# arindamrc/video_analytics

Hardware: AMD Instinct MI355X
Metric: clips/sec (224x224, RGB+10-flow two-stream) (higher is better)
Workload: dtype f32; 1 GPU; two-stream 224x224, 10-frame TV-L1 flow stack (5 scales x 5 warps x 300 its, fixed), VGG-16 spatial+temporal, batch=32 per GPU; global_batch=32, block_iters=0, tvl1_math=exact, flow_streams=2, batches_in_flight=1, tvl1_params=, tvl1_hip_blob=08077c666a7db564113fbd6e9b9134d85ffd8245, parallelism=clips sharded x1, finite=True

## Files before the change

video_analytics_amd/csrc/tvl1.hip:

```cpp
#include "va_internal.h"
#include <cmath>
#include <algorithm>
#include <cstdlib>
#include <cstring>
#include <utility>
#include <type_traits>

namespace {

constexpr int kNF_STATE = 6;
constexpr int kNF_RO = 4;


__device__ __forceinline__ void bilinear3_shfl(const float* __restrict__ I1, size_t plane, int w, int h, int pitch, float x,
                                               float y, bool active, float& v0, float& v1, float& v2)
{
    x = fminf(fmaxf(x, 0.0f), (float)(w - 1));
    y = fminf(fmaxf(y, 0.0f), (float)(h - 1));
    const int x0 = (int)x, y0 = (int)y;
    const int x1 = d_min(x0 + 1, w - 1), y1 = d_min(y0 + 1, h - 1);
    const float ax = x - (float)x0, ay = y - (float)y0;
    const int o00 = y0 * pitch + x0, o10 = y1 * pitch + x0;
    float a[3], c[3], b[3], d[3];
#pragma unroll
// ... 30 lines not shown
    v2 = r[2];
}

__global__ void k_warp(const float* __restrict__ pyr, size_t plane, int w, int h, int pitch, int fps,
                       const float* __restrict__ stA, const float* __restrict__ stB, const int* __restrict__ sel, int cur,
                       int* __restrict__ base, float* __restrict__ ro, int pair0, int perm)
{
    unsigned lid = blockIdx.y * gridDim.x + blockIdx.x;
    {
        const unsigned nb = gridDim.x * gridDim.y, q = nb / 8, r = nb % 8, xcd = lid % 8, kk = lid / 8;
        lid = (xcd < r ? xcd * (q + 1) : r * (q + 1) + (xcd - r) * q) + kk;
    }
    const int pair = pair0 + (int)(lid / gridDim.x);
    const int idx = (int)(lid % gridDim.x) * blockDim.x + threadIdx.x;
    const int which = sel ? sel[pair] : cur;
    if (base && idx == 0) base[pair] = which;
    const bool active = idx < w * h;
    const int y = active ? idx / w : 0, x = active ? idx - y * w : 0;
    const int seq = pair / (fps - 1), k = pair - seq * (fps - 1);
    const int f0 = seq * fps + k;
    const float* I0 = pyr + (size_t)f0 * 3 * plane;
    const float* I1 = pyr + (size_t)(f0 + 1) * 3 * plane;
    const float* st = (which ? stB : stA) + (size_t)pair * kNF_STATE * plane;
    const size_t o = (size_t)y * pitch + x, op = (size_t)y * pitch + pslot(x, perm);
    const float u1 = active ? st[op] : 0.0f, u2 = active ? st[plane + op] : 0.0f;
    float Iw, Iwx, Iwy;
    bilinear3_shfl(I1, plane, w, h, pitch, (float)x + u1, (float)y + u2, active, Iw, Iwx, Iwy);
    if (!active) return;
    const float grad = fmaf(Iwy, Iwy, Iwx * Iwx);
    float* r = ro + (size_t)pair * kNF_RO * plane;
    r[op] = Iwx;
    r[plane + op] = Iwy;
    r[2 * plane + op] = fmaf(-Iwy, u2, fmaf(-Iwx, u1, Iw - I0[o]));
    r[3 * plane + op] = grad < 1e-10f ? 0.0f : 1.0f / grad;
}

__global__ void k_upsample(const float* __restrict__ stA, const float* __restrict__ stB, const int* __restrict__ sel,
                           int cur, int cw, int ch, int cpitch, size_t cplane, float* __restrict__ tmp, int fw, int fh,
                           int fpitch, size_t fplane, float inv_step, int cperm)
{
    const int pair = blockIdx.y;
    const int idx = blockIdx.x * blockDim.x + threadIdx.x;
    if (idx >= fw * fh) return;
    const int which = sel ? sel[pair] : cur;
    const float* src = (which ? stB : stA) + (size_t)pair * kNF_STATE * cplane;
    float* dst = tmp + (size_t)pair * 2 * fplane;
    const int y = idx / fw, x = idx - y * fw;
    const float rx = (float)cw / (float)fw, ry = (float)ch / (float)fh;
    const size_t o = (size_t)y * fpitch + x;
    dst[o] = bilinear(src, cw, ch, cpitch, (float)x * rx, (float)y * ry, cperm) * inv_step;
    dst[fplane + o] = bilinear(src + cplane, cw, ch, cpitch, (float)x * rx, (float)y * ry, cperm) * inv_step;
}

__global__ void k_level_init(const float* __restrict__ tmp, float* __restrict__ st0, int w, int h, int pitch, size_t plane, int perm)
{
    const int pair = blockIdx.y;
    const int idx = blockIdx.x * blockDim.x + threadIdx.x;
    if (idx >= pitch * h) return;
    const int y = idx / pitch, x = idx - y * pitch;
    const size_t o = (size_t)y * pitch + x, op = (size_t)y * pitch + pslot(x, perm);
    const float* t = tmp + (size_t)pair * 2 * plane;
    float* dst = st0 + (size_t)pair * kNF_STATE * plane;
    dst[op] = x < w ? t[o] : 0.0f;
    dst[plane + op] = x < w ? t[plane + o] : 0.0f;
    dst[2 * plane + op] = 0.0f;
    dst[3 * plane + op] = 0.0f;
    dst[4 * plane + op] = 0.0f;
    dst[5 * plane + op] = 0.0f;
}

__global__ void k_zero_pad(float* __restrict__ buf, int nf, int w, int h, int pitch, size_t plane, int perm)
{
    const int pair = blockIdx.y, pw = pitch - w;
    const int idx = blockIdx.x * blockDim.x + threadIdx.x;
    if (idx >= pw * h * nf) return;
    const int f = idx / (pw * h), r = idx - f * pw * h, y = r / pw, x = w + r - y * pw;
    buf[((size_t)pair * nf + f) * plane + (size_t)y * pitch + pslot(x, perm)] = 0.0f;
}

__global__ void k_flow_out(const float* __restrict__ stA, const float* __restrict__ stB, const int* __restrict__ sel,
                           int cur, int w, int h, int pitch, size_t plane, float* __restrict__ flow, int perm)
{
    const int pair = blockIdx.y;
    const int idx = blockIdx.x * blockDim.x + threadIdx.x;
    if (idx >= w * h) return;
    const int which = sel ? sel[pair] : cur;
    const float* st = (which ? stB : stA) + (size_t)pair * kNF_STATE * plane;
    const int y = idx / w, x = idx - y * w;
    flow[((size_t)pair * 2) * w * h + idx] = st[(size_t)y * pitch + pslot(x, perm)];
    flow[((size_t)pair * 2 + 1) * w * h + idx] = st[plane + (size_t)y * pitch + pslot(x, perm)];
}

__global__ void k_flow_to_stack(const float* __restrict__ flow, float* __restrict__ stack, size_t n, float bound,
                                float mean, float stdv)
{
    const size_t i = (size_t)blockIdx.x * blockDim.x + threadIdx.x;
    if (i >= n) return;
    const float t = (255.0f * (flow[i] + bound)) / (2.0f * bound);
    const float q = rintf(fminf(fmaxf(t, 0.0f), 255.0f));
    stack[i] = (q / 255.0f - mean) / stdv;
}


struct IterArgs {
    const float* ro;
    const float* stA;
    const float* stB;
    float* outA;
    float* outB;
    const int* base;
    int* sel;
    unsigned long long* err;
    unsigned long long qthr;
// ... 387 lines not shown
    float prev = dpp_from_left(row_get(a, N - 1));
#pragma clang loop unroll(full)
    for (int i = 0; i < N; ++i) {
        const float cur = row_get(a, i);
        row_set(d, i, i == 0 ? cur - prev : sub_s(cur, prev));
        prev = cur;
    }
    return d;
}
template <int N>
__device__ __forceinline__ Row<N> r_diff_fwd(const Row<N>& a)
{
    Row<N> d;
    d.t = 0.0f;
    const float right = dpp_from_right(row_get(a, 0));
#pragma clang loop unroll(full)
    for (int i = 0; i < N; ++i)
        row_set(d, i, i < N - 1 ? sub_s(row_get(a, i + 1 < N ? i + 1 : 0), row_get(a, i)) : right - row_get(a, i));
    return d;
}

template <int PPL> struct RowIo;
template <> struct RowIo<2> {
    typedef unsigned V __attribute__((ext_vector_type(2)));
    static __device__ __forceinline__ V ld(__amdgpu_buffer_rsrc_t r, int vo, int so) { return __builtin_amdgcn_raw_buffer_load_b64(r, vo, so, 0); }
    static __device__ __forceinline__ void st(V v, __amdgpu_buffer_rsrc_t r, int vo, int so) { __builtin_amdgcn_raw_buffer_store_b64(v, r, vo, so, 0); }
};
template <int N>
__device__ __forceinline__ Row<N> row_load(__amdgpu_buffer_rsrc_t r, int vo, int so)
{
    const typename RowIo<N>::V v = RowIo<N>::ld(r, vo, so);
    Row<N> o;
    o.t = 0.0f;
#pragma clang loop unroll(full)
    for (int i = 0; i < N; ++i) row_set(o, i, __uint_as_float(v[i]));
    return o;
}
template <int N>
__device__ __forceinline__ void row_store(const Row<N>& o, __amdgpu_buffer_rsrc_t r, int vo, int so)
{
    typename RowIo<N>::V v;
#pragma clang loop unroll(full)
    for (int i = 0; i < N; ++i) v[i] = __float_as_uint(row_get(o, i));
    RowIo<N>::st(v, r, vo, so);
}


struct StreamArgs {
    const float* ro;
    const float* sin;
    float* sout;
    size_t plane;
    int w, h, pitch;
    int nsx, nch, R, HX;
    int K;
    int pair0, rev;
    float l_t, taut, theta;
    int narrow, npairs;
};

template <int KH, int NCH>
struct StreamShape {
    static_assert(KH % NCH == 0, "the levels of a wave are cut into chains of equal length");
    static constexpr int KC = KH / NCH;
    static constexpr int SPAN = KH + NCH;
    static constexpr int lpos(int t) { return t + t / KC; }
// ... 19 lines not shown
    typedef StreamRow<PPL> SR;
    typedef StreamShape<KH, NCH> SH;
    constexpr int NP = R::NP, NT = R::NT, SW = 64 * PPL, KC = SH::KC;
    constexpr int NRING = stream_ring_rows<KH, NWV, NCH>() > 0 ? stream_ring_rows<KH, NWV, NCH>() : 1;
    typedef float f4 __attribute__((ext_vector_type(4)));
    static_assert(kNF_RO % 2 == 0 && kNF_STATE % 2 == 0, "fields pair up into 16-byte units");
    __shared__ f4 ringP[NRING][kNF_RO / 2][NP][64];
    __shared__ float ringT[NRING][kNF_RO][NT ? 64 : 1];
    __shared__ f4 ifaceP[NWV > 1 ? NWV - 1 : 1][2][kNF_STATE / 2][NP][64];
    __shared__ float ifaceT[NWV > 1 ? NWV - 1 : 1][2][kNF_STATE][NT ? 64 : 1];

    const int sx = job % a.nsx, ch = job / a.nsx;
    const int w = a.w, h = a.h, pitch = a.pitch;
    const int lane = threadIdx.x & 63;
    const int wv = NWV == 1 ? 0 : __builtin_amdgcn_readfirstlane((int)(threadIdx.x >> 6));
    const int ox = sx * (SW - 2 * a.HX);
    const int vx0 = ox + (sx > 0 ? a.HX : 0), vx1 = (sx == a.nsx - 1) ? pitch : ox + SW - a.HX;
    const int x0 = ox + PPL * (half ? (lane & 31) : lane);
    const bool colok = x0 < pitch && !(half == 2 && lane >= 32);
    const bool stok = colok && x0 >= vx0 && x0 < vx1;
    const int a0 = ch * a.R, b0 = d_min(h, a0 + a.R);
    const int ys = d_max(0, a0 - K), ye = d_min(h, b0 + K);

    const int planeb = (int)(a.plane * sizeof(float)), pitchb = pitch * (int)sizeof(float);
    const int npr = half == 1 ? 2 : 1;
    const __amdgpu_buffer_rsrc_t rs_ro = __builtin_amdgcn_make_buffer_rsrc(
        const_cast<float*>(a.ro + (size_t)pair * kNF_RO * a.plane), 0, npr * kNF_RO * planeb, 0x00020000);
    const __amdgpu_buffer_rsrc_t rs_in = __builtin_amdgcn_make_buffer_rsrc(
        const_cast<float*>(sin_all + (size_t)pair * kNF_STATE * a.plane), 0, npr * kNF_STATE * planeb, 0x00020000);
    const __amdgpu_buffer_rsrc_t rs_out = __builtin_amdgcn_make_buffer_rsrc(sout_all + (size_t)pair * kNF_STATE * a.plane, 0,
                                                                           npr * kNF_STATE * planeb, 0x00020000);
    const bool second = half == 1 && lane >= 32;
    const int loff = colok ? x0 * (int)sizeof(float) + (second ? kNF_STATE * planeb : 0) : 0;
    const int loff_ro = colok ? x0 * (int)sizeof(float) + (second ? kNF_RO * planeb : 0) : 0;

    R mx;
    mx.t = 0.0f;
#pragma clang loop unroll(full)
    for (int i = 0; i < PPL; ++i) row_set(mx, i, x0 + i < w - 1 ? 1.0f : 0.0f);
    const float l_t = a.l_t, taut = a.taut, theta = a.theta;
    const R zero = row_splat<PPL>(0.0f), one = row_splat<PPL>(1.0f);

    auto unit_put = [&](f4 (*u)[64], float (*t)[NT ? 64 : 1], int f, const R& v0, const R& v1) __attribute__((always_inline)) {
#pragma clang loop unroll(full)
        for (int j = 0; j < NP; ++j) u[j][lane] = f4{v0.p[j].x, v0.p[j].y, v1.p[j].x, v1.p[j].y};
        if constexpr (NT) {
            t[f][lane] = v0.t;
            t[f + 1][lane] = v1.t;
        }
    };
    auto unit_get = [&](const f4 (*u)[64], const float (*t)[NT ? 64 : 1], int f, R& v0, R& v1) __attribute__((always_inline)) {
#pragma clang loop unroll(full)
        for (int j = 0; j < NP; ++j) {
            const f4 q = u[j][lane];
            v0.p[j] = f2{q.x, q.y};
            v1.p[j] = f2{q.z, q.w};
        }
// ... 15 lines not shown
        unit_put(ifaceP[wb][b][0], ifaceT[wb][b], 0, v.u1, v.u2);
        unit_put(ifaceP[wb][b][1], ifaceT[wb][b], 2, v.p11, v.p12);
        unit_put(ifaceP[wb][b][2], ifaceT[wb][b], 4, v.p21, v.p22);
    };
    auto if_get = [&](int wb, int b, SR& v) __attribute__((always_inline)) {
        unit_get(ifaceP[wb][b][0], ifaceT[wb][b], 0, v.u1, v.u2);
        unit_get(ifaceP[wb][b][1], ifaceT[wb][b], 2, v.p11, v.p12);
        unit_get(ifaceP[wb][b][2], ifaceT[wb][b], 4, v.p21, v.p22);
    };

    {
        const R zro[kNF_RO] = {zero, zero, zero, zero};
        for (int r = wv; r < NRING; r += NWV) ring_put(r, zro);
    }
    if constexpr (NWV > 1) {
        if (wv < NWV - 1) {
            const SR zst{zero, zero, zero, zero, zero, zero};
            if_put(wv, 0, zst);
            if_put(wv, 1, zst);
        }
        __syncthreads();
    }

    auto ld = [&](const __amdgpu_buffer_rsrc_t& r, int f, int y) -> R { return row_load<PPL>(r, loff, f * planeb + y * pitchb); };
    auto ld_ro = [&](int f, int y) -> R { return row_load<PPL>(rs_ro, loff_ro, f * planeb + y * pitchb); };
    auto st = [&](const R& v, int f, int y) { row_store<PPL>(v, rs_out, loff, f * planeb + y * pitchb); };

    const int nsteps = b0 - ys + K + (NWV * NCH - 1);

    auto run = [&](auto wave_tag, auto mx1_tag) __attribute__((always_inline)) {
        constexpr int W = decltype(wave_tag)::value;
        constexpr bool MX1 = decltype(mx1_tag)::value;
        constexpr bool FIRST = W == 0, LAST = W == NWV - 1;
        constexpr int G0 = W * KH, LAG = W * SH::SPAN;

        R P11[KH], P12[KH], P21[KH], P22[KH], U1[KH], U2[KH];
#pragma clang loop unroll(full)
        for (int t = 0; t < KH; ++t) P11[t] = P12[t] = P21[t] = P22[t] = U1[t] = U2[t] = zero;
        SR latch[NCH > 1 ? NCH - 1 : 1];
#pragma clang loop unroll(full)
        for (int c = 0; c < (NCH > 1 ? NCH - 1 : 1); ++c) latch[c] = SR{zero, zero, zero, zero, zero, zero};
        R nst[kNF_STATE], nro[kNF_RO], rprev[kNF_RO] = {zero, zero, zero, zero};
        constexpr bool KEEP = LAST && stream_keep_last<KH, NWV, NCH>();
        R keep[kNF_RO] = {zero, zero, zero, zero};
#pragma clang loop unroll(full)
        for (int f = 0; f < kNF_STATE; ++f) nst[f] = FIRST ? ld(rs_in, f, ys) : zero;
#pragma clang loop unroll(full)
        for (int f = 0; f < kNF_RO; ++f) nro[f] = FIRST ? ld_ro(f, ys) : zero;

        auto level = [&](int t, SR& c, const R& wx, const R& wy, const R& rc, const R& ig, const float my, auto my1_tag) __attribute__((always_inline)) {
            constexpr bool MY1 = decltype(my1_tag)::value;
            const R dx11 = r_diff_back(c.p11), dx21 = r_diff_back(c.p21);
            const R div1 = r_add(dx11, r_sub(c.p12, P12[t]));
            const R div2 = r_add(dx21, r_sub(c.p22, P22[t]));
            const R rho = r_fma(wy, c.u2, r_fma(wx, c.u1, rc));
            const R tt = r_negmul(rho, ig);
            const R fi = r_med3(tt, -l_t, l_t);
            const R v1 = r_fma(fi, wx, c.u1);
            const R v2 = r_fma(fi, wy, c.u2);
            const R n1 = r_fma_s(theta, div1, v1);
            const R n2 = r_fma_s(theta, div2, v2);
            const R d1x = r_diff_fwd(U1[t]), d2x = r_diff_fwd(U2[t]);
            const R u1x = MX1 ? d1x : r_mul(d1x, mx), u1y = MY1 ? r_sub(n1, U1[t]) : r_mul_s(r_sub(n1, U1[t]), my);
            const R u2x = MX1 ? d2x : r_mul(d2x, mx), u2y = MY1 ? r_sub(n2, U2[t]) : r_mul_s(r_sub(n2, U2[t]), my);
            const R s1 = r_fma(u1y, u1y, r_fma_c(u1x, u1x, kSqrtReg));
            const R s2 = r_fma(u2y, u2y, r_fma_c(u2x, u2x, kSqrtReg));
            const R d1 = r_fma_s(taut, r_sqrt<PPL, FAST>(s1), one);
            const R d2 = r_fma_s(taut, r_sqrt<PPL, FAST>(s2), one);
            R q1, q2;
            if constexpr (FAST) {
                q1 = r_rcp<PPL, true>(d1);
// ... 13 lines not shown
            P21[t] = c.p21;
            P22[t] = c.p22;
            U1[t] = n1;
            U2[t] = n2;
            c.u1 = ou1;
            c.u2 = ou2;
            c.p11 = o11;
            c.p12 = o12;
            c.p21 = o21;
            c.p22 = o22;
        };

        auto step = [&](const int s, auto steady_tag) __attribute__((always_inline)) {
            constexpr bool STEADY = decltype(steady_tag)::value;
            const int s0 = s % NRING;
            SR cc[NCH];
            R r0[kNF_RO] = {zero, zero, zero, zero};
            if constexpr (FIRST) {
                cc[0] = SR{nst[0], nst[1], nst[2], nst[3], nst[4], nst[5]};
#pragma clang loop unroll(full)
                for (int f = 0; f < kNF_RO; ++f) r0[f] = nro[f];
                const int rn = d_min(ys + s + 1, ye - 1);
#pragma clang loop unroll(full)
                for (int f = 0; f < kNF_STATE; ++f) nst[f] = ld(rs_in, f, rn);
#pragma clang loop unroll(full)
                for (int f = 0; f < kNF_RO; ++f) nro[f] = ld_ro(f, rn);
                if constexpr (NWV > 1) {
                    const int sl = s0 == 0 ? NRING - 1 : s0 - 1;
                    ring_put(sl, rprev);
                }
                __builtin_amdgcn_sched_barrier(0);
            } else {
                const int bsel = (s + 1) & 1;
                if_get(W - 1, bsel, cc[0]);
            }
#pragma clang loop unroll(full)
            for (int c = 1; c < NCH; ++c) cc[c] = latch[c - 1];
            auto slot_of = [&](int t) {
                const int c = (LAG + SH::lpos(t)) % NRING;
                return s0 - c < 0 ? s0 - c + NRING : s0 - c;
            };
            if constexpr (STEADY) {
                R q[NCH][kNF_RO];
#pragma clang loop unroll(full)
                for (int c = 0; c < NCH; ++c) {
                    if (FIRST && c == 0) {
#pragma clang loop unroll(full)
                        for (int f = 0; f < kNF_RO; ++f) q[c][f] = r0[f];
                    } else {
// ... 39 lines not shown
                    if (act) {
                        const float my = rin - 1 < h - 1 ? 1.0f : 0.0f;
                        if (FIRST && t == 0) {
                            level(0, cc[0], r0[0], r0[1], r0[2], r0[3], my, std::false_type{});
                        } else if (KEEP && t == KH - 1) {
                            level(t, cc[t / KC], keep[0], keep[1], keep[2], keep[3], my, std::false_type{});
                        } else {
                            R q[kNF_RO];
                            ring_get(slot_of(t), q);
                            level(t, cc[t / KC], q[0], q[1], q[2], q[3], my, std::false_type{});
                        }
                    }
                }
                if constexpr (KEEP) {
                    ring_get(slot_of(KH - 2), keep);
                }
            }
#pragma clang loop unroll(full)
            for (int c = 0; c + 1 < NCH; ++c) latch[c] = cc[c];
            const SR& co = cc[NCH - 1];
            if constexpr (LAST) {
                const int rout = ys + s - K - (NWV * NCH - 1);
                if (stok && rout >= a0 && rout < b0) {
                    st(co.u1, 0, rout);
                    st(co.u2, 1, rout);
                    st(co.p11, 2, rout);
                    st(co.p12, 3, rout);
                    st(co.p21, 4, rout);
                    st(co.p22, 5, rout);
                }
            } else {
                if_put(W, s & 1, co);
            }
            if constexpr (FIRST) {
                if constexpr (NWV == 1) {
                    ring_put(s0, r0);
                } else {
#pragma clang loop unroll(full)
                    for (int f = 0; f < kNF_RO; ++f) rprev[f] = r0[f];
                }
            }
            if constexpr (NWV > 1) asm volatile("s_waitcnt lgkmcnt(0)\n\ts_barrier" ::: "memory");
        };
        int s_a = 0, s_b = nsteps;
#pragma clang loop unroll(full)
        for (int t = 0; t < KH; ++t) {
            const int g = G0 + t, p = LAG + SH::lpos(t) - ys;
            s_a = d_max(s_a, d_max(0, a0 - (K - g)) + p);
            s_b = d_min(s_b, d_min(h - 1, d_min(h, b0 + (K - g) - 1)) + p + 1);
        }
        if (K < G0 + KH || s_a > s_b) s_a = s_b = 0;
        int s = 0;
        for (; s < s_a; ++s) step(s, std::false_type{});
        if constexpr (NWV > 1)
            for (; s + 1 < s_b; s += 2) {
                step(s, std::true_type{});
                step(s + 1, std::true_type{});
            }
        for (; s < s_b; ++s) step(s, std::true_type{});
        for (; s < nsteps; ++s) step(s, std::false_type{});
    };
    auto waves = [&](auto mx1_tag) __attribute__((always_inline)) {
        if constexpr (NWV == 1) {
            run(std::integral_constant<int, 0>{}, mx1_tag);
        } else if constexpr (NWV == 2) {
            if (wv == 0) run(std::integral_constant<int, 0>{}, mx1_tag);
            else run(std::integral_constant<int, NWV - 1>{}, mx1_tag);
        } else if constexpr (NWV == 3) {
            if (wv == 0) run(std::integral_constant<int, 0>{}, mx1_tag);
            else if (wv == 1) run(std::integral_constant<int, 1>{}, mx1_tag);
            else run(std::integral_constant<int, 2>{}, mx1_tag);
        } else {
            static_assert(NWV == 4, "pipelines of one to four waves");
            if (wv == 0) run(std::integral_constant<int, 0>{}, mx1_tag);
            else if (wv == 1) run(std::integral_constant<int, 1>{}, mx1_tag);
            else if (wv == 2) run(std::integral_constant<int, 2>{}, mx1_tag);
            else run(std::integral_constant<int, 3>{}, mx1_tag);
        }
    };
    if constexpr (kStreamMx1<KH, NWV>) {
        if (half == 0 && ox + SW < w) waves(std::true_type{});
        else waves(std::false_type{});
// ... 76 lines not shown
    size_t plane;
    int src_nf, dst_nf;
    int cur, it, iters;
    int w, h, pitch, perm, ntx, pair0;
};

constexpr int kMedTX = 64, kMedTY = 16, kMedRows = 4;

__device__ __forceinline__ int median_buffer(const MedianArgs& a, int pair)
{
    if (!a.err) return a.cur;
    if (a.it > 0 && a.err[(size_t)pair * a.iters + a.it - 1] < a.qthr) return -1;
    return a.base[pair] ^ (a.it & 1);
}

template <int KS>
__global__ void __launch_bounds__(kMedTX * (kMedTY / kMedRows)) k_median(MedianArgs a)
{
    constexpr int R = KS / 2, LW = kMedTX + 2 * R, LH = kMedTY + 2 * R, NT = kMedTX * (kMedTY / kMedRows);
    __shared__ float tile[LH][LW];
    const int pair = a.pair0 + blockIdx.y, f = blockIdx.z;
    const int which = median_buffer(a, pair);
    if (which < 0) return;
    const float* __restrict__ src = (which ? a.srcB : a.srcA) + ((size_t)pair * a.src_nf + f) * a.plane;
    float* __restrict__ dst = (which ? a.dstB : a.dstA) + ((size_t)pair * a.dst_nf + f) * a.plane;
    const int w = a.w, h = a.h, pitch = a.pitch, perm = a.perm;
    const int ox = (int)(blockIdx.x % a.ntx) * kMedTX, oy = (int)(blockIdx.x / a.ntx) * kMedTY;
    const int tid = threadIdx.y * kMedTX + threadIdx.x;
    for (int i = tid; i < LW * LH; i += NT) {
        const int ly = i / LW, lx = i - ly * LW;
        const int gx = d_min(d_max(ox + lx - R, 0), w - 1), gy = d_min(d_max(oy + ly - R, 0), h - 1);
        tile[ly][lx] = src[(size_t)gy * pitch + pslot(gx, perm)];
    }
    __syncthreads();
    const int x = ox + threadIdx.x;
    if (x >= w) return;
    for (int j = 0; j < kMedRows; ++j) {
        const int ly = threadIdx.y * kMedRows + j, y = oy + ly;
        if (y >= h) break;
        float v[KS * KS];
#pragma unroll
        for (int dy = 0; dy < KS; ++dy)
#pragma unroll
            for (int dx = 0; dx < KS; ++dx) v[dy * KS + dx] = tile[ly + dy][threadIdx.x + dx];
        dst[(size_t)y * pitch + pslot(x, perm)] = median_of<KS * KS>(v);
    }
}

__global__ void k_median_store(MedianArgs a)
{
    const int pair = a.pair0 + blockIdx.y, f = blockIdx.z;
    const int idx = blockIdx.x * blockDim.x + threadIdx.x;
    if (idx >= a.w * a.h) return;
    const int which = median_buffer(a, pair);
    if (which < 0) return;
    const float* __restrict__ src = (which ? a.srcB : a.srcA) + ((size_t)pair * a.src_nf + f) * a.plane;
    float* __restrict__ dst = (which ? a.dstB : a.dstA) + ((size_t)pair * a.dst_nf + f) * a.plane;
    const int y = idx / a.w, x = idx - y * a.w;
    const size_t o = (size_t)y * a.pitch + pslot(x, a.perm);
    dst[o] = src[o];
}

dim3 median_grid(const MedianArgs& a, int npairs) { return dim3(a.ntx * va_cdiv(a.h, kMedTY), npairs, 2); }
void launch_median(int ksize, const MedianArgs& a, int npairs, hipStream_t st)
{
    const dim3 grid = median_grid(a, npairs), block(kMedTX, kMedTY / kMedRows);
    if (ksize == 3) k_median<3><<<grid, block, 0, st>>>(a);
    else k_median<5><<<grid, block, 0, st>>>(a);
}


struct TileCfg {
    int R, C, NW, LX;
};
constexpr TileCfg kCfgs[] = {{4, 4, 8, 64}, {4, 4, 8, 32}, {4, 4, 8, 21}, {4, 4, 8, 16},
                             {4, 4, 4, 64}, {4, 4, 4, 32}, {4, 4, 4, 21}, {4, 4, 4, 16}};
constexpr int kNumCfgs = (int)(sizeof(kCfgs) / sizeof(kCfgs[0]));

struct TilePick {
    int cfg, ntx, nty, HX, K;
};

// ... 287 lines not shown
               const LevelBufs& B, hipStream_t st, LaunchLog* log, int* cur_out)
{
    float* const* pyr = B.pyr;
    float* const tmp1 = B.tmp1;
    float* const state[2] = {B.state[0], B.state[1]};
    float* const ro = B.ro;
    unsigned long long* const err = B.err;
    int* const sel = B.sel;
    int* const base = B.base;
    const bool eps = p->epsilon > 0.0f;
    const bool prof = live && ctx->prof_on;
    const int TPB = 256;
    const int sc = P.ns - 1;
    int cur = 0;
    int K0 = p->block_iters;
    if (eps) K0 = 1;

    for (int s = sc; s >= 0; --s) {
        const int lw = P.ws[s], lh = P.hs[s], lp = P.pitch[s];
        const size_t plane = P.plane[s];
        const unsigned tmask = (unsigned)p->tile_mask & (unsigned)(kStreamBit - 1);
        const TilePick tp = K0 > 0 ? pick_tiles(lw, lh, K0, tmask) : pick_tiles_auto(lw, lh, median ? median_every : p->iters, tmask);
        const bool strm = P.lk[s] == LK_STREAM;
        const int perm = strm ? 0 : 1;
        if (live && lp != lw) {
            k_zero_pad<<<dim3(va_cdiv((lp - lw) * lh * kNF_RO, TPB), P.NP), TPB, 0, st>>>(ro, kNF_RO, lw, lh, lp, plane, perm);
            VA_LAUNCH_CHECK();
        }
        const int cp = (eps || strm) ? P.NP : chunk_pairs(lw, lh, tp, P.NP);
        const int cur_in = cur;
        for (int c0 = 0; c0 < P.NP; c0 += cp) {
            const int nc = P.NP - c0 < cp ? P.NP - c0 : cp;
            const dim3 gpc(va_cdiv(lw * lh, TPB), nc);
            cur = cur_in;
            for (int wp = 0; wp < p->warps; ++wp) {
                if (live) {
                    k_warp<<<gpc, TPB, 0, st>>>(pyr[s], plane, lw, lh, lp, P.F, state[0], state[1], eps ? sel : nullptr, cur,
                                                 eps ? base : nullptr, ro, c0, perm);
                    VA_LAUNCH_CHECK();
                    if (eps) VA_HIP(hipMemsetAsync(err, 0, (size_t)P.NP * p->iters * sizeof(unsigned long long), st));
                }
                va_prof_span span{};
                if (prof) {
                    span = prof_get(ctx);
                    span.level = s;
                    VA_HIP(hipEventRecord(span.beg, st));
                }
// ... 196 lines not shown
                        const int n = p->iters - it0 < median_every ? p->iters - it0 : median_every;
                        if (int rc = run_iters(it0, n)) return rc;
                    }
                }
                if (live) VA_LAUNCH_CHECK();
                if (prof) {
                    VA_HIP(hipEventRecord(span.end, st));
                    ctx->prof_spans.push_back(span);
                    ctx->prof_launches += launches;
                    ctx->prof_pxiters += (double)nc * lw * lh * p->iters;
                    ctx->prof_pxwarps += (double)nc * lw * lh;
                    if (s < kVaProfLevels) {
                        ctx->prof_level_pxiters[s] += (double)nc * lw * lh * p->iters;
                        ctx->prof_level_launches[s] += launches;
                    }
                }
            }
        }
        if (s > 0) {
            if (live) {
                const dim3 g(va_cdiv(P.ws[s - 1] * P.hs[s - 1], TPB), P.NP);
                k_upsample<<<g, TPB, 0, st>>>(state[0], state[1], eps ? sel : nullptr, cur, lw, lh, lp, plane, ro, P.ws[s - 1],
                                               P.hs[s - 1], P.pitch[s - 1], P.plane[s - 1], 1.0f / p->scale_step, perm);
                const int fperm = P.lk[s - 1] != LK_TILE ? 0 : 1;
                const dim3 gi(va_cdiv(P.pitch[s - 1] * P.hs[s - 1], TPB), P.NP);
                k_level_init<<<gi, TPB, 0, st>>>(ro, state[0], P.ws[s - 1], P.hs[s - 1], P.pitch[s - 1], P.plane[s - 1], fperm);
                VA_LAUNCH_CHECK();
            }
            cur = 0;
            if (live && eps) VA_HIP(hipMemsetAsync(sel, 0, (size_t)P.NP * sizeof(int), st));
        }
    }
    *cur_out = cur;
    return VA_OK;
}

}

extern "C" void va_tvl1_default_params(va_tvl1_params* p)
{
    if (!p) return;
    p->tau = 0.25f;
    p->lambda = 0.15f;
    p->theta = 0.3f;
    p->nscales = 5;
    p->warps = 5;
    p->epsilon = 0.01f;
// ... 121 lines not shown

    if (int rc = va_stage_frames(frames, frames_are_u8, false, pyr[0], w, h, P.pitch[0], P.plane[0], P.NF, st)) return rc;
    if (int rc = va_stage_pyramid(pyr, P.ws, P.hs, P.pitch, P.plane, P.ns, P.NF, tmp1, tmp2, P.plane_max, p->scale_step, st)) return rc;
    for (int s = 0; s < P.ns; ++s)
        if (int rc = va_stage_gradient(pyr[s], P.ws[s], P.hs[s], P.pitch[s], P.plane[s], P.NF, st)) return rc;

    const int sc = P.ns - 1;
    VA_HIP(hipMemsetAsync(state[0], 0, (size_t)P.NP * kNF_STATE * P.plane[sc] * sizeof(float), st));
    VA_HIP(hipMemsetAsync(sel, 0, (size_t)P.NP * 2 * sizeof(int), st));
    int cur = 0;
    LevelBufs B{};
    for (int s = 0; s < P.ns; ++s) B.pyr[s] = pyr[s];
    B.tmp1 = tmp1;
    B.state[0] = state[0];
    B.state[1] = state[1];
    B.ro = ro;
    B.err = err;
    B.sel = sel;
    B.base = base;
    if (int rc = run_levels(ctx, true, P, p, median, median_every, B, st, nullptr, &cur)) return rc;
    {
        const dim3 g(va_cdiv(w * h, TPB), P.NP);
        k_flow_out<<<g, TPB, 0, st>>>(state[0], state[1], eps ? sel : nullptr, cur, w, h, P.pitch[0], P.plane[0], (float*)flow,
                                       P.lk[0] != LK_TILE ? 0 : 1);
        VA_LAUNCH_CHECK();
    }
    return VA_OK;
}

extern "C" int va_flow_to_stack(va_ctx* ctx, const void* flow, int n_pairs, int w, int h, float bound, float mean,
                                float stdv, void* stack, void* stream)
{
    VA_CHECK_ARG(ctx != nullptr, "va_flow_to_stack: ctx is NULL");
    VA_USE_DEVICE(ctx);
    VA_CHECK_ARG(flow != nullptr && stack != nullptr, "va_flow_to_stack: NULL buffer");
    VA_CHECK_ARG(n_pairs >= 1 && w >= 1 && h >= 1, "va_flow_to_stack: bad shape");
    VA_CHECK_ARG(bound > 0.0f && stdv > 0.0f, "va_flow_to_stack: bound and std must be > 0");
    const size_t n = (size_t)n_pairs * 2 * w * h;
    k_flow_to_stack<<<(unsigned)((n + 255) / 256), 256, 0, (hipStream_t)stream>>>((const float*)flow, (float*)stack, n, bound, mean, stdv);
    VA_LAUNCH_CHECK();
    return VA_OK;
}

extern "C" int va_flow_median(va_ctx* ctx, const void* flow, int n_fields, int w, int h, int ksize, void* out, void* stream)
{
    VA_CHECK_ARG(ctx != nullptr, "va_flow_median: ctx is NULL");
    VA_USE_DEVICE(ctx);
// ... 86 lines not shown
    if (reset) ctx->prof_ms = ctx->prof_union_ms = ctx->prof_launches = ctx->prof_pxiters = ctx->prof_pxwarps = 0.0;
    return VA_OK;
}

extern "C" int va_tvl1_profile_levels(va_ctx* ctx, double* out, int n, int reset)
{
    VA_CHECK_ARG(ctx != nullptr && out != nullptr && n >= 1 && n <= kVaProfLevels, "va_tvl1_profile_levels: bad argument");
    for (int s = 0; s < n; ++s) {
        out[3 * s + 0] = ctx->prof_level_ms[s];
        out[3 * s + 1] = ctx->prof_level_pxiters[s];
        out[3 * s + 2] = ctx->prof_level_launches[s];
    }
    if (reset)
        for (int s = 0; s < kVaProfLevels; ++s) ctx->prof_level_ms[s] = ctx->prof_level_pxiters[s] = ctx->prof_level_launches[s] = 0.0;
    return VA_OK;
}


int va_stage_upsample(const float* cstate, int cw, int ch, int cpitch, size_t cplane, float* tmp, float* fstate, int fw, int fh,
                      int fpitch, size_t fplane, float inv_step, int NP, hipStream_t st)
{
    const int TPB = 256;
    k_upsample<<<dim3(va_cdiv(fw * fh, TPB), NP), TPB, 0, st>>>(cstate, cstate, nullptr, 0, cw, ch, cpitch, cplane, tmp, fw, fh, fpitch,
                                                                 fplane, inv_step, 0);
    k_level_init<<<dim3(va_cdiv(fpitch * fh, TPB), NP), TPB, 0, st>>>(tmp, fstate, fw, fh, fpitch, fplane, 0);
    VA_LAUNCH_CHECK();
    return VA_OK;
}

int va_stage_flow_out(const float* state, int w, int h, int pitch, size_t plane, float* flow, int NP, hipStream_t st)
{
    k_flow_out<<<dim3(va_cdiv(w * h, 256), NP), 256, 0, st>>>(state, state, nullptr, 0, w, h, pitch, plane, flow, 0);
    VA_LAUNCH_CHECK();
    return VA_OK;
}
```

video_analytics_amd/csrc/va_internal.h:

```cpp
#pragma once
#include <hip/hip_runtime.h>
#include <cstdarg>
#include <cstdio>
#include <vector>
#include "../../include/va.h"

struct va_prof_span {
    hipEvent_t beg, end;
    int level;
};
constexpr int kVaProfLevels = 16;

struct va_ctx {
    int device;
    int n_cu;
    bool prof_on;
    std::vector<va_prof_span> prof_spans;
    std::vector<va_prof_span> prof_pool;
    hipEvent_t prof_ref;
    double prof_ms, prof_union_ms, prof_launches, prof_pxiters, prof_pxwarps;
    double prof_level_ms[kVaProfLevels], prof_level_pxiters[kVaProfLevels], prof_level_launches[kVaProfLevels];
};

void va_set_error(const char* fmt, ...);
// ... 89 lines not shown
struct va_carver {
    void* base;
    size_t off = 0;
    template <class T>
    T* take(size_t count)
    {
        T* p = (T*)((uintptr_t)base + off);
        off += va_align_up(count * sizeof(T), 256);
        return p;
    }
};

int va_integral_planes(const unsigned* votes, unsigned* out, long long planes, int w, int h, hipStream_t st);


constexpr int kVaMaxScales = 16;
constexpr int kVaMaxLds = 160 * 1024;

__device__ __forceinline__ int d_min(int a, int b) { return a < b ? a : b; }
__device__ __forceinline__ int d_max(int a, int b) { return a > b ? a : b; }

__device__ __forceinline__ int pslot(int x, int perm) { return perm ? ((x & ~3) | ((x & 1) << 1) | ((x >> 1) & 1)) : x; }

__device__ __forceinline__ float bilinear(const float* __restrict__ img, int w, int h, int pitch, float x, float y, int perm = 0)
{
    x = fminf(fmaxf(x, 0.0f), (float)(w - 1));
    y = fminf(fmaxf(y, 0.0f), (float)(h - 1));
    const int x0 = (int)x, y0 = (int)y;
    const int x1 = d_min(x0 + 1, w - 1), y1 = d_min(y0 + 1, h - 1);
    const float ax = x - (float)x0, ay = y - (float)y0;
    const int s0 = pslot(x0, perm), s1 = pslot(x1, perm);
    const float a = img[y0 * pitch + s0], b = img[y0 * pitch + s1];
    const float c = img[y1 * pitch + s0], d = img[y1 * pitch + s1];
    const float top = fmaf(ax, b - a, a);
    const float bot = fmaf(ax, d - c, c);
    return fmaf(ay, bot - top, top);
}

template <typename K>
int va_allow_lds(K* kernel, size_t lds)
{
    if (lds > 64 * 1024) VA_HIP(hipFuncSetAttribute(reinterpret_cast<const void*>(kernel), hipFuncAttributeMaxDynamicSharedMemorySize, kVaMaxLds));
    return VA_OK;
}

struct va_flow_levels {
    int ns, ws[kVaMaxScales], hs[kVaMaxScales], pitch[kVaMaxScales];
    size_t plane[kVaMaxScales], plane_max;
    int F, NF, NP;
};
int va_flow_pyramid_sizes(int w, int h, float scale_step, int nscales, int* ws, int* hs);
void va_flow_levels_fill(va_flow_levels* L, int w, int h, int n_seq, int fps, float scale_step, int nscales);

int va_flow_check_shape(const char* who, int w, int h, int n_seq, int fps, bool frames);
int va_flow_check_fields(const char* who, int n, int w, int h);
int va_flow_check_buffers(const char* who, const void* frames, const void* flow, const void* workspace, size_t have, size_t need);

void va_stage_layout(int w, int h, int* pitch, size_t* plane);
int va_stage_frames(const void* frames, int frames_are_u8, bool unit_range, float* pyr0, int w, int h, int pitch, size_t plane, int NF,
// ... 50 lines not shown
```

Before: 268.7 clips/s.

## Interleave field pairs per row so streaming TV-L1 kernel uses 128-bit buffer loads

Introduces a paired-row layout for the streaming TV-L1 levels in which two fields (u1/u2, p11/p12, p21/p22, and the ro pairs) share a row with their pixels interleaved. The streaming kernel can then fetch and store two fields with one 128-bit buffer op instead of two 64-bit ops, halving the memory instruction count in the inner loop. Every helper kernel (warp, upsample, level init, zero pad, median, flow out) is rewritten to address through a common field_slot function. It also adds a priority reset after each store and drops the unpaired tail loop when NWV>1. The risks are broader access strides and possible layout mismatches between the helper kernels and the streaming kernel.

```diff
diff --git a/video_analytics_amd/csrc/tvl1.hip b/video_analytics_amd/csrc/tvl1.hip
--- a/video_analytics_amd/csrc/tvl1.hip
+++ b/video_analytics_amd/csrc/tvl1.hip
@@ -76,17 +76,18 @@
     const float* I0 = pyr + (size_t)f0 * 3 * plane;
     const float* I1 = pyr + (size_t)(f0 + 1) * 3 * plane;
     const float* st = (which ? stB : stA) + (size_t)pair * kNF_STATE * plane;
-    const size_t o = (size_t)y * pitch + x, op = (size_t)y * pitch + pslot(x, perm);
-    const float u1 = active ? st[op] : 0.0f, u2 = active ? st[plane + op] : 0.0f;
+    const size_t o = (size_t)y * pitch + x;
+    auto op = [&](int f) { return field_slot(f, y, x, pitch, plane, perm); };
+    const float u1 = active ? st[op(0)] : 0.0f, u2 = active ? st[op(1)] : 0.0f;
     float Iw, Iwx, Iwy;
     bilinear3_shfl(I1, plane, w, h, pitch, (float)x + u1, (float)y + u2, active, Iw, Iwx, Iwy);
     if (!active) return;
     const float grad = fmaf(Iwy, Iwy, Iwx * Iwx);
     float* r = ro + (size_t)pair * kNF_RO * plane;
-    r[op] = Iwx;
-    r[plane + op] = Iwy;
-    r[2 * plane + op] = fmaf(-Iwy, u2, fmaf(-Iwx, u1, Iw - I0[o]));
-    r[3 * plane + op] = grad < 1e-10f ? 0.0f : 1.0f / grad;
+    r[op(0)] = Iwx;
+    r[op(1)] = Iwy;
+    r[op(2)] = fmaf(-Iwy, u2, fmaf(-Iwx, u1, Iw - I0[o]));
+    r[op(3)] = grad < 1e-10f ? 0.0f : 1.0f / grad;
 }
 
 __global__ void k_upsample(const float* __restrict__ stA, const float* __restrict__ stB, const int* __restrict__ sel,
@@ -102,8 +103,8 @@
     const int y = idx / fw, x = idx - y * fw;
     const float rx = (float)cw / (float)fw, ry = (float)ch / (float)fh;
     const size_t o = (size_t)y * fpitch + x;
-    dst[o] = bilinear(src, cw, ch, cpitch, (float)x * rx, (float)y * ry, cperm) * inv_step;
-    dst[fplane + o] = bilinear(src + cplane, cw, ch, cpitch, (float)x * rx, (float)y * ry, cperm) * inv_step;
+    dst[o] = bilinear_field(src, 0, cw, ch, cpitch, cplane, (float)x * rx, (float)y * ry, cperm) * inv_step;
+    dst[fplane + o] = bilinear_field(src, 1, cw, ch, cpitch, cplane, (float)x * rx, (float)y * ry, cperm) * inv_step;
 }
 
 __global__ void k_level_init(const float* __restrict__ tmp, float* __restrict__ st0, int w, int h, int pitch, size_t plane, int perm)
@@ -112,15 +113,16 @@
     const int idx = blockIdx.x * blockDim.x + threadIdx.x;
     if (idx >= pitch * h) return;
     const int y = idx / pitch, x = idx - y * pitch;
-    const size_t o = (size_t)y * pitch + x, op = (size_t)y * pitch + pslot(x, perm);
+    const size_t o = (size_t)y * pitch + x;
+    auto op = [&](int f) { return field_slot(f, y, x, pitch, plane, perm); };
     const float* t = tmp + (size_t)pair * 2 * plane;
     float* dst = st0 + (size_t)pair * kNF_STATE * plane;
-    dst[op] = x < w ? t[o] : 0.0f;
-    dst[plane + op] = x < w ? t[plane + o] : 0.0f;
-    dst[2 * plane + op] = 0.0f;
-    dst[3 * plane + op] = 0.0f;
-    dst[4 * plane + op] = 0.0f;
-    dst[5 * plane + op] = 0.0f;
+    dst[op(0)] = x < w ? t[o] : 0.0f;
+    dst[op(1)] = x < w ? t[plane + o] : 0.0f;
+    dst[op(2)] = 0.0f;
+    dst[op(3)] = 0.0f;
+    dst[op(4)] = 0.0f;
+    dst[op(5)] = 0.0f;
 }
 
 __global__ void k_zero_pad(float* __restrict__ buf, int nf, int w, int h, int pitch, size_t plane, int perm)
@@ -129,7 +131,7 @@
     const int idx = blockIdx.x * blockDim.x + threadIdx.x;
     if (idx >= pw * h * nf) return;
     const int f = idx / (pw * h), r = idx - f * pw * h, y = r / pw, x = w + r - y * pw;
-    buf[((size_t)pair * nf + f) * plane + (size_t)y * pitch + pslot(x, perm)] = 0.0f;
+    buf[(size_t)pair * nf * plane + field_slot(f, y, x, pitch, plane, perm)] = 0.0f;
 }
 
 __global__ void k_flow_out(const float* __restrict__ stA, const float* __restrict__ stB, const int* __restrict__ sel,
@@ -141,8 +143,8 @@
     const int which = sel ? sel[pair] : cur;
     const float* st = (which ? stB : stA) + (size_t)pair * kNF_STATE * plane;
     const int y = idx / w, x = idx - y * w;
-    flow[((size_t)pair * 2) * w * h + idx] = st[(size_t)y * pitch + pslot(x, perm)];
-    flow[((size_t)pair * 2 + 1) * w * h + idx] = st[plane + (size_t)y * pitch + pslot(x, perm)];
+    flow[((size_t)pair * 2) * w * h + idx] = st[field_slot(0, y, x, pitch, plane, perm)];
+    flow[((size_t)pair * 2 + 1) * w * h + idx] = st[field_slot(1, y, x, pitch, plane, perm)];
 }
 
 __global__ void k_flow_to_stack(const float* __restrict__ flow, float* __restrict__ stack, size_t n, float bound,
@@ -576,26 +578,30 @@
 
 template <int PPL> struct RowIo;
 template <> struct RowIo<2> {
-    typedef unsigned V __attribute__((ext_vector_type(2)));
-    static __device__ __forceinline__ V ld(__amdgpu_buffer_rsrc_t r, int vo, int so) { return __builtin_amdgcn_raw_buffer_load_b64(r, vo, so, 0); }
-    static __device__ __forceinline__ void st(V v, __amdgpu_buffer_rsrc_t r, int vo, int so) { __builtin_amdgcn_raw_buffer_store_b64(v, r, vo, so, 0); }
+    typedef unsigned V __attribute__((ext_vector_type(4)));
+    static __device__ __forceinline__ V ld(__amdgpu_buffer_rsrc_t r, int vo, int so) { return __builtin_amdgcn_raw_buffer_load_b128(r, vo, so, 0); }
+    static __device__ __forceinline__ void st(V v, __amdgpu_buffer_rsrc_t r, int vo, int so) { __builtin_amdgcn_raw_buffer_store_b128(v, r, vo, so, 0); }
 };
 template <int N>
-__device__ __forceinline__ Row<N> row_load(__amdgpu_buffer_rsrc_t r, int vo, int so)
+__device__ __forceinline__ void row_load2(Row<N>& f0, Row<N>& f1, __amdgpu_buffer_rsrc_t r, int vo, int so)
 {
     const typename RowIo<N>::V v = RowIo<N>::ld(r, vo, so);
-    Row<N> o;
-    o.t = 0.0f;
-#pragma clang loop unroll(full)
-    for (int i = 0; i < N; ++i) row_set(o, i, __uint_as_float(v[i]));
-    return o;
+    f0.t = f1.t = 0.0f;
+#pragma clang loop unroll(full)
+    for (int i = 0; i < N; ++i) {
+        row_set(f0, i, __uint_as_float(v[i]));
+        row_set(f1, i, __uint_as_float(v[N + i]));
+    }
 }
 template <int N>
-__device__ __forceinline__ void row_store(const Row<N>& o, __amdgpu_buffer_rsrc_t r, int vo, int so)
+__device__ __forceinline__ void row_store2(const Row<N>& f0, const Row<N>& f1, __amdgpu_buffer_rsrc_t r, int vo, int so)
 {
     typename RowIo<N>::V v;
 #pragma clang loop unroll(full)
-    for (int i = 0; i < N; ++i) v[i] = __float_as_uint(row_get(o, i));
+    for (int i = 0; i < N; ++i) {
+        v[i] = __float_as_uint(row_get(f0, i));
+        v[N + i] = __float_as_uint(row_get(f1, i));
+    }
     RowIo<N>::st(v, r, vo, so);
 }
 
@@ -661,7 +667,8 @@
     const int a0 = ch * a.R, b0 = d_min(h, a0 + a.R);
     const int ys = d_max(0, a0 - K), ye = d_min(h, b0 + K);
 
-    const int planeb = (int)(a.plane * sizeof(float)), pitchb = pitch * (int)sizeof(float);
+    static_assert(PPL == 2, "a lane slot of the paired row layout holds two pixels of two fields");
+    const int planeb = (int)(a.plane * sizeof(float)), prowb = 2 * pitch * (int)sizeof(float);
     const int npr = half == 1 ? 2 : 1;
     const __amdgpu_buffer_rsrc_t rs_ro = __builtin_amdgcn_make_buffer_rsrc(
         const_cast<float*>(a.ro + (size_t)pair * kNF_RO * a.plane), 0, npr * kNF_RO * planeb, 0x00020000);
@@ -670,8 +677,9 @@
     const __amdgpu_buffer_rsrc_t rs_out = __builtin_amdgcn_make_buffer_rsrc(sout_all + (size_t)pair * kNF_STATE * a.plane, 0,
                                                                            npr * kNF_STATE * planeb, 0x00020000);
     const bool second = half == 1 && lane >= 32;
-    const int loff = colok ? x0 * (int)sizeof(float) + (second ? kNF_STATE * planeb : 0) : 0;
-    const int loff_ro = colok ? x0 * (int)sizeof(float) + (second ? kNF_RO * planeb : 0) : 0;
+    const int slotb = (int)(field_slot(0, 0, x0, pitch, a.plane, kRowsPaired) * sizeof(float));
+    const int loff = colok ? slotb + (second ? kNF_STATE * planeb : 0) : 0;
+    const int loff_ro = colok ? slotb + (second ? kNF_RO * planeb : 0) : 0;
 
     R mx;
     mx.t = 0.0f;
@@ -733,9 +741,14 @@
         __syncthreads();
     }
 
-    auto ld = [&](const __amdgpu_buffer_rsrc_t& r, int f, int y) -> R { return row_load<PPL>(r, loff, f * planeb + y * pitchb); };
-    auto ld_ro = [&](int f, int y) -> R { return row_load<PPL>(rs_ro, loff_ro, f * planeb + y * pitchb); };
-    auto st = [&](const R& v, int f, int y) { row_store<PPL>(v, rs_out, loff, f * planeb + y * pitchb); };
+    auto ld = [&](const __amdgpu_buffer_rsrc_t& r, R& v0, R& v1, int f, int y) { row_load2<PPL>(v0, v1, r, loff, f * planeb + y * prowb); };
+    auto ld_ro = [&](R& v0, R& v1, int f, int y) { row_load2<PPL>(v0, v1, rs_ro, loff_ro, f * planeb + y * prowb); };
+    auto st = [&](const R& v0, const R& v1, int f, int y) {
+        row_store2<PPL>(v0, v1, rs_out, loff, f * planeb + y * prowb);
+        __builtin_amdgcn_sched_barrier(0);
+        __builtin_amdgcn_s_setprio(0);
+        __builtin_amdgcn_sched_barrier(0);
+    };
 
     const int nsteps = b0 - ys + K + (NWV * NCH - 1);
 
@@ -755,9 +768,15 @@
         constexpr bool KEEP = LAST && stream_keep_last<KH, NWV, NCH>();
         R keep[kNF_RO] = {zero, zero, zero, zero};
 #pragma clang loop unroll(full)
-        for (int f = 0; f < kNF_STATE; ++f) nst[f] = FIRST ? ld(rs_in, f, ys) : zero;
-#pragma clang loop unroll(full)
-        for (int f = 0; f < kNF_RO; ++f) nro[f] = FIRST ? ld_ro(f, ys) : zero;
+        for (int f = 0; f < kNF_STATE; ++f) nst[f] = zero;
+#pragma clang loop unroll(full)
+        for (int f = 0; f < kNF_RO; ++f) nro[f] = zero;
+        if constexpr (FIRST) {
+#pragma clang loop unroll(full)
+            for (int f = 0; f < kNF_STATE; f += 2) ld(rs_in, nst[f], nst[f + 1], f, ys);
+#pragma clang loop unroll(full)
+            for (int f = 0; f < kNF_RO; f += 2) ld_ro(nro[f], nro[f + 1], f, ys);
+        }
 
         auto level = [&](int t, SR& c, const R& wx, const R& wy, const R& rc, const R& ig, const float my, auto my1_tag) __attribute__((always_inline)) {
             constexpr bool MY1 = decltype(my1_tag)::value;
@@ -817,9 +836,9 @@
                 for (int f = 0; f < kNF_RO; ++f) r0[f] = nro[f];
                 const int rn = d_min(ys + s + 1, ye - 1);
 #pragma clang loop unroll(full)
-                for (int f = 0; f < kNF_STATE; ++f) nst[f] = ld(rs_in, f, rn);
-#pragma clang loop unroll(full)
-                for (int f = 0; f < kNF_RO; ++f) nro[f] = ld_ro(f, rn);
+                for (int f = 0; f < kNF_STATE; f += 2) ld(rs_in, nst[f], nst[f + 1], f, rn);
+#pragma clang loop unroll(full)
+                for (int f = 0; f < kNF_RO; f += 2) ld_ro(nro[f], nro[f + 1], f, rn);
                 if constexpr (NWV > 1) {
                     const int sl = s0 == 0 ? NRING - 1 : s0 - 1;
                     ring_put(sl, rprev);
@@ -905,12 +924,9 @@
             if constexpr (LAST) {
                 const int rout = ys + s - K - (NWV * NCH - 1);
                 if (stok && rout >= a0 && rout < b0) {
-                    st(co.u1, 0, rout);
-                    st(co.u2, 1, rout);
-                    st(co.p11, 2, rout);
-                    st(co.p12, 3, rout);
-                    st(co.p21, 4, rout);
-                    st(co.p22, 5, rout);
+                    st(co.u1, co.u2, 0, rout);
+                    st(co.p11, co.p12, 2, rout);
+                    st(co.p21, co.p22, 4, rout);
                 }
             } else {
                 if_put(W, s & 1, co);
@@ -935,12 +951,14 @@
         if (K < G0 + KH || s_a > s_b) s_a = s_b = 0;
         int s = 0;
         for (; s < s_a; ++s) step(s, std::false_type{});
-        if constexpr (NWV > 1)
+        if constexpr (NWV > 1) {
             for (; s + 1 < s_b; s += 2) {
                 step(s, std::true_type{});
                 step(s + 1, std::true_type{});
             }
-        for (; s < s_b; ++s) step(s, std::true_type{});
+        } else {
+            for (; s < s_b; ++s) step(s, std::true_type{});
+        }
         for (; s < nsteps; ++s) step(s, std::false_type{});
     };
     auto waves = [&](auto mx1_tag) __attribute__((always_inline)) {
@@ -1063,15 +1081,15 @@
     const int pair = a.pair0 + blockIdx.y, f = blockIdx.z;
     const int which = median_buffer(a, pair);
     if (which < 0) return;
-    const float* __restrict__ src = (which ? a.srcB : a.srcA) + ((size_t)pair * a.src_nf + f) * a.plane;
-    float* __restrict__ dst = (which ? a.dstB : a.dstA) + ((size_t)pair * a.dst_nf + f) * a.plane;
+    const float* __restrict__ src = (which ? a.srcB : a.srcA) + (size_t)pair * a.src_nf * a.plane;
+    float* __restrict__ dst = (which ? a.dstB : a.dstA) + (size_t)pair * a.dst_nf * a.plane;
     const int w = a.w, h = a.h, pitch = a.pitch, perm = a.perm;
     const int ox = (int)(blockIdx.x % a.ntx) * kMedTX, oy = (int)(blockIdx.x / a.ntx) * kMedTY;
     const int tid = threadIdx.y * kMedTX + threadIdx.x;
     for (int i = tid; i < LW * LH; i += NT) {
         const int ly = i / LW, lx = i - ly * LW;
         const int gx = d_min(d_max(ox + lx - R, 0), w - 1), gy = d_min(d_max(oy + ly - R, 0), h - 1);
-        tile[ly][lx] = src[(size_t)gy * pitch + pslot(gx, perm)];
+        tile[ly][lx] = src[field_slot(f, gy, gx, pitch, a.plane, perm)];
     }
     __syncthreads();
     const int x = ox + threadIdx.x;
@@ -1084,7 +1102,7 @@
         for (int dy = 0; dy < KS; ++dy)
 #pragma unroll
             for (int dx = 0; dx < KS; ++dx) v[dy * KS + dx] = tile[ly + dy][threadIdx.x + dx];
-        dst[(size_t)y * pitch + pslot(x, perm)] = median_of<KS * KS>(v);
+        dst[field_slot(f, y, x, pitch, a.plane, perm)] = median_of<KS * KS>(v);
     }
 }
 
@@ -1095,10 +1113,10 @@
     if (idx >= a.w * a.h) return;
     const int which = median_buffer(a, pair);
     if (which < 0) return;
-    const float* __restrict__ src = (which ? a.srcB : a.srcA) + ((size_t)pair * a.src_nf + f) * a.plane;
-    float* __restrict__ dst = (which ? a.dstB : a.dstA) + ((size_t)pair * a.dst_nf + f) * a.plane;
+    const float* __restrict__ src = (which ? a.srcB : a.srcA) + (size_t)pair * a.src_nf * a.plane;
+    float* __restrict__ dst = (which ? a.dstB : a.dstA) + (size_t)pair * a.dst_nf * a.plane;
     const int y = idx / a.w, x = idx - y * a.w;
-    const size_t o = (size_t)y * a.pitch + pslot(x, a.perm);
+    const size_t o = field_slot(f, y, x, a.pitch, a.plane, a.perm);
     dst[o] = src[o];
 }
 
@@ -1432,7 +1450,7 @@
         const unsigned tmask = (unsigned)p->tile_mask & (unsigned)(kStreamBit - 1);
         const TilePick tp = K0 > 0 ? pick_tiles(lw, lh, K0, tmask) : pick_tiles_auto(lw, lh, median ? median_every : p->iters, tmask);
         const bool strm = P.lk[s] == LK_STREAM;
-        const int perm = strm ? 0 : 1;
+        const int perm = strm ? kRowsPaired : kRowsTile;
         if (live && lp != lw) {
             k_zero_pad<<<dim3(va_cdiv((lp - lw) * lh * kNF_RO, TPB), P.NP), TPB, 0, st>>>(ro, kNF_RO, lw, lh, lp, plane, perm);
             VA_LAUNCH_CHECK();
@@ -1675,7 +1693,7 @@
                 const dim3 g(va_cdiv(P.ws[s - 1] * P.hs[s - 1], TPB), P.NP);
                 k_upsample<<<g, TPB, 0, st>>>(state[0], state[1], eps ? sel : nullptr, cur, lw, lh, lp, plane, ro, P.ws[s - 1],
                                                P.hs[s - 1], P.pitch[s - 1], P.plane[s - 1], 1.0f / p->scale_step, perm);
-                const int fperm = P.lk[s - 1] != LK_TILE ? 0 : 1;
+                const int fperm = P.lk[s - 1] != LK_TILE ? kRowsPaired : kRowsTile;
                 const dim3 gi(va_cdiv(P.pitch[s - 1] * P.hs[s - 1], TPB), P.NP);
                 k_level_init<<<gi, TPB, 0, st>>>(ro, state[0], P.ws[s - 1], P.hs[s - 1], P.pitch[s - 1], P.plane[s - 1], fperm);
                 VA_LAUNCH_CHECK();
@@ -1843,7 +1861,7 @@
     {
         const dim3 g(va_cdiv(w * h, TPB), P.NP);
         k_flow_out<<<g, TPB, 0, st>>>(state[0], state[1], eps ? sel : nullptr, cur, w, h, P.pitch[0], P.plane[0], (float*)flow,
-                                       P.lk[0] != LK_TILE ? 0 : 1);
+                                       P.lk[0] != LK_TILE ? kRowsPaired : kRowsTile);
         VA_LAUNCH_CHECK();
     }
     return VA_OK;
@@ -1976,15 +1994,15 @@
 {
     const int TPB = 256;
     k_upsample<<<dim3(va_cdiv(fw * fh, TPB), NP), TPB, 0, st>>>(cstate, cstate, nullptr, 0, cw, ch, cpitch, cplane, tmp, fw, fh, fpitch,
-                                                                 fplane, inv_step, 0);
-    k_level_init<<<dim3(va_cdiv(fpitch * fh, TPB), NP), TPB, 0, st>>>(tmp, fstate, fw, fh, fpitch, fplane, 0);
+                                                                 fplane, inv_step, kRowsPlain);
+    k_level_init<<<dim3(va_cdiv(fpitch * fh, TPB), NP), TPB, 0, st>>>(tmp, fstate, fw, fh, fpitch, fplane, kRowsPlain);
     VA_LAUNCH_CHECK();
     return VA_OK;
 }
 
 int va_stage_flow_out(const float* state, int w, int h, int pitch, size_t plane, float* flow, int NP, hipStream_t st)
 {
-    k_flow_out<<<dim3(va_cdiv(w * h, 256), NP), 256, 0, st>>>(state, state, nullptr, 0, w, h, pitch, plane, flow, 0);
+    k_flow_out<<<dim3(va_cdiv(w * h, 256), NP), 256, 0, st>>>(state, state, nullptr, 0, w, h, pitch, plane, flow, kRowsPlain);
     VA_LAUNCH_CHECK();
     return VA_OK;
 }
diff --git a/video_analytics_amd/csrc/va_internal.h b/video_analytics_amd/csrc/va_internal.h
--- a/video_analytics_amd/csrc/va_internal.h
+++ b/video_analytics_amd/csrc/va_internal.h
@@ -135,19 +135,35 @@
 
 __device__ __forceinline__ int pslot(int x, int perm) { return perm ? ((x & ~3) | ((x & 1) << 1) | ((x >> 1) & 1)) : x; }
 
-__device__ __forceinline__ float bilinear(const float* __restrict__ img, int w, int h, int pitch, float x, float y, int perm = 0)
+constexpr int kRowsPlain = 0, kRowsTile = 1, kRowsPaired = 2;
+__device__ __forceinline__ size_t field_slot(int f, int y, int x, int pitch, size_t plane, int perm)
+{
+    if (perm == kRowsPaired) return (size_t)(f >> 1) * 2 * plane + (size_t)y * 2 * pitch + (((x >> 1) << 2) | ((f & 1) << 1) | (x & 1));
+    return (size_t)f * plane + (size_t)y * pitch + pslot(x, perm);
+}
+
+template <typename Tap>
+__device__ __forceinline__ float bilinear_taps(int w, int h, float x, float y, Tap tap)
 {
     x = fminf(fmaxf(x, 0.0f), (float)(w - 1));
     y = fminf(fmaxf(y, 0.0f), (float)(h - 1));
     const int x0 = (int)x, y0 = (int)y;
     const int x1 = d_min(x0 + 1, w - 1), y1 = d_min(y0 + 1, h - 1);
     const float ax = x - (float)x0, ay = y - (float)y0;
-    const int s0 = pslot(x0, perm), s1 = pslot(x1, perm);
-    const float a = img[y0 * pitch + s0], b = img[y0 * pitch + s1];
-    const float c = img[y1 * pitch + s0], d = img[y1 * pitch + s1];
+    const float a = tap(x0, y0), b = tap(x1, y0);
+    const float c = tap(x0, y1), d = tap(x1, y1);
     const float top = fmaf(ax, b - a, a);
     const float bot = fmaf(ax, d - c, c);
     return fmaf(ay, bot - top, top);
+}
+__device__ __forceinline__ float bilinear(const float* __restrict__ img, int w, int h, int pitch, float x, float y)
+{
+    return bilinear_taps(w, h, x, y, [&](int xi, int yi) { return img[yi * pitch + xi]; });
+}
+__device__ __forceinline__ float bilinear_field(const float* __restrict__ fields, int f, int w, int h, int pitch, size_t plane, float x,
+                                                float y, int perm)
+{
+    return bilinear_taps(w, h, x, y, [&](int xi, int yi) { return fields[field_slot(f, yi, xi, pitch, plane, perm)]; });
 }
 
 template <typename K>
```

Measured after the change: 269.0 clips/s, median of 2. No clear change (+0.1%).
